# abmoRobotics/isaac_rover_2.0

Hardware: AMD Instinct MI355X
Metric: env-steps/sec (obs+reward+done) (higher is better)
Workload: dtype f32; 1 GPU; BASELINE configs[2]: 65536 envs/GPU x 1 GPU, 37-point heightmap + 26 rock rays, K=200, 600x600 cells @0.1 m, stone_info mask over 1024 stones, cell_index_mode=cuda_rcp; envs_total=65536, rays_per_env=63, obs_dim=41, algorithmic_bytes_per_env_step=227148

## Files before the change

isaac_rover_2.0_amd/csrc/rover_kernels.hip:

```cpp
#include <hip/hip_runtime.h>
#include <stdint.h>
#include <type_traits>
#include "rover_internal.h"
#include "rover_philox.h"
#include "rover_raymath.h"

namespace rover {


__device__ __forceinline__ float quat_roll(const float* __restrict__ q) {
    float w = q[0], x = q[1], y = q[2], z = q[3];
    float sinr = 2.0f * (w * x + y * z);
    float cosr = 1.0f - (2.0f * (x * x + y * y));
    return atan2f(sinr, cosr);
}
__device__ __forceinline__ float quat_pitch(const float* __restrict__ q) {
    const float half_pi = 3.1415927410125732f / 2.0f;
    float w = q[0], x = q[1], y = q[2], z = q[3];
    float sinp = 2.0f * (w * y - z * x);
    float t = sinp - 1.0f;
    return (t >= 0.0f) ? copysignf(half_pi, sinp) : asinf(sinp);
}
__device__ __forceinline__ float quat_yaw(const float* __restrict__ q) {
    float w = q[0], x = q[1], y = q[2], z = q[3];
// ... 736 lines not shown
    float alpha = (float)(2 * 3.14159265358979323846) * u;
    float gx = radius * cosf(alpha) + 0.0f, gy = radius * sinf(alpha) + 0.0f;
    x = gx + initial_pos3[3ull * id];
    y = gy + initial_pos3[3ull * id + 1];
}

__device__ __forceinline__ float height_at(const HeightDev& h, float x, float y) {
    uint32_t ix = cell_coord(x, h.shift_x, h.hscale, h.inv_hscale, h.rcp, h.N0);
    uint32_t iy = cell_coord(y, h.shift_y, h.hscale, h.inv_hscale, h.rcp, h.N0);
    if (iy > (uint32_t)(h.N1 - 1)) iy = (uint32_t)(h.N1 - 1);
    return h.hm[(uint64_t)ix * h.N1 + iy] * h.vscale;
}

#define GOAL_LANES 8u

__global__ void __launch_bounds__(256) goals_draw_kernel(GoalArgs a) {
    const uint32_t n = a.n_dev ? (uint32_t)max(*a.n_dev, 0) : a.n_host;
    const uint32_t gt = blockIdx.x * 256u + threadIdx.x;
    const uint32_t i = gt / GOAL_LANES, j = gt % GOAL_LANES;
    const uint32_t shift = (threadIdx.x & 63u) & ~(GOAL_LANES - 1u);
    const bool live = i < n;
    const int64_t id = live ? a.env_ids[i] - a.id_offset : 0;
    if (live && id == 0 && j == 0) a.t_acc[i] = -1;
    bool active = live && id != 0;
    for (int32_t t0 = 0; t0 < a.max_draws; t0 += (int32_t)GOAL_LANES) {
        if (__builtin_amdgcn_ballot_w64(active) == 0) break;
        const int32_t t = t0 + (int32_t)j;
        bool clear = false;
        float x = 0.0f, y = 0.0f;
        if (active && t < a.max_draws) {
            float u = a.draws ? a.draws[(uint64_t)t * n + i] : philox_uniform(a.seed + (a.seed_dev ? *a.seed_dev : 0ull), (uint32_t)t, (uint32_t)a.env_ids[i]);
            goal_from_draw(u, a.radius, a.initial_pos3, id, x, y);
            clear = !collides_grid(a.grid, a.info7, x, y, 1.0f);
        }
        const uint32_t m = (uint32_t)(__builtin_amdgcn_ballot_w64(clear) >> shift) & ((1u << GOAL_LANES) - 1u);
        if (active) {
            const bool last_trip = t0 + (int32_t)GOAL_LANES >= a.max_draws;
            int32_t winner = -1;
            if (m) winner = (int32_t)__builtin_ctz(m);
            else if (last_trip) winner = a.max_draws - 1 - t0;
            if (winner >= 0) {
                if ((int32_t)j == winner) {
                    a.t_acc[i] = m ? t : a.max_draws;
                    a.target3[3ull * id] = x; a.target3[3ull * id + 1] = y;
                    a.target3[3ull * id + 2] = height_at(a.h, x, y);
                }
                active = false;
            }
        }
    }
}

__global__ void __launch_bounds__(1024) goals_env0_kernel(GoalArgs a) {
    __shared__ int s_tmax, s_lz, s_has_zero, s_fail;
    const uint32_t tid = threadIdx.x;
    const uint32_t n = a.n_dev ? (uint32_t)max(*a.n_dev, 0) : a.n_host;
    if (n == 0) { if (tid == 0 && a.n_draws_used) *a.n_draws_used = 0; return; }
    if (tid == 0) { s_tmax = -1; s_lz = -1; s_has_zero = 0; s_fail = 0; }
    __syncthreads();
    int my_tmax = -1;
    bool my_zero = false, my_fail = false;
    for (uint32_t i = tid; i < n; i += blockDim.x) {
        int32_t t = a.t_acc[i];
        if (t >= a.max_draws) my_fail = true;
        else if (t < 0) my_zero = true;
        else my_tmax = max(my_tmax, t);
    }
#pragma unroll
    for (int o = 32; o >= 1; o >>= 1) my_tmax = max(my_tmax, __shfl_xor(my_tmax, o));
    const bool w_zero = __builtin_amdgcn_ballot_w64(my_zero) != 0, w_fail = __builtin_amdgcn_ballot_w64(my_fail) != 0;
    if ((tid & 63u) == 0u) {
        if (my_tmax >= 0) atomicMax(&s_tmax, my_tmax);
        if (w_zero) s_has_zero = 1;
        if (w_fail) s_fail = 1;
    }
    __syncthreads();
    if (s_fail) { if (tid == 0 && a.n_draws_used) *a.n_draws_used = -1; return; }
    const int tmax = s_tmax;
    int my_lz = -1;
    for (uint32_t i = tid; i < n; i += blockDim.x) {
        int32_t t = a.t_acc[i];
        if (t < 0 || t < tmax) my_lz = max(my_lz, (int)i);
    }
#pragma unroll
    for (int o = 32; o >= 1; o >>= 1) my_lz = max(my_lz, __shfl_xor(my_lz, o));
    if ((tid & 63u) == 0u && my_lz >= 0) atomicMax(&s_lz, my_lz);
    __syncthreads();
    if (tid >= 64u) return;
    const int32_t t0 = max(tmax, 0);
    const int lz0 = s_lz;
    int32_t used = -1;
    float x = 0.0f, y = 0.0f;
    bool wrote = false;
    if (lz0 < 0) {
        used = t0 + 1;
    } else {
        for (int32_t base = t0; base < a.max_draws; base += 64) {
            const int32_t t = base + (int32_t)tid;
            const uint32_t src = (t == t0) ? (uint32_t)lz0 : n - 1u;
            bool clear = false;
            float cx = 0.0f, cy = 0.0f;
            if (t < a.max_draws) {
                float u = a.draws ? a.draws[(uint64_t)t * n + src] : philox_uniform(a.seed + (a.seed_dev ? *a.seed_dev : 0ull), (uint32_t)t, (uint32_t)a.env_ids[src]);
                goal_from_draw(u, a.radius, a.initial_pos3, 0, cx, cy);
                clear = !collides_grid(a.grid, a.info7, cx, cy, 1.0f);
            }
            const uint64_t m = __builtin_amdgcn_ballot_w64(clear);
            const bool last_trip = base + 64 >= a.max_draws;
            int32_t winner = -1;
            if (m) winner = (int32_t)__builtin_ctzll(m);
            else if (last_trip) winner = a.max_draws - 1 - base;
            if (winner >= 0) {
                x = __shfl(cx, winner); y = __shfl(cy, winner);
                wrote = true;
                if (m) used = base + winner + 1;
                break;
            }
        }
    }
    if (tid != 0) return;
    if (wrote) {
        a.target3[0] = x; a.target3[1] = y;
        if (s_has_zero) a.target3[2] = height_at(a.h, x, y);
    }
    if (a.n_draws_used) *a.n_draws_used = used;
}

__global__ void __launch_bounds__(256) reset_envs_kernel(ResetArgs a) {
    const uint32_t n = a.n_dev ? (uint32_t)max(*a.n_dev, 0) : a.n_host;
    uint32_t i = blockIdx.x * blockDim.x + threadIdx.x;
    if (i >= n) return;
    const int64_t id = a.ids[i] - a.id_offset;
    float deg = a.yaw_deg ? (float)a.yaw_deg[i]
                          : floorf(philox_uniform((a.seed + (a.seed_dev ? *a.seed_dev : 0ull)) ^ 0x9E3779B97F4A7C15ull, 0u, (uint32_t)a.ids[i]) * 361.0f);
    float half = (deg * (3.14159265358979323846f / 180.0f)) / 2.0f;
    a.quat4[4ull * id] = sinf(half); a.quat4[4ull * id + 1] = 0.0f; a.quat4[4ull * id + 2] = 0.0f; a.quat4[4ull * id + 3] = cosf(half);
#pragma unroll
    for (int c = 0; c < 3; ++c) {
        float v = a.initial_pos3[3ull * id + c];
        a.pos3[3ull * id + c] = v;
        if (a.base_pos3) a.base_pos3[3ull * id + c] = v;
    }
    for (int j = 0; j < 13; ++j) {
        if (a.joint_pos13) a.joint_pos13[13ull * id + j] = 0.0f;
        if (a.joint_vel13) a.joint_vel13[13ull * id + j] = 0.0f;
    }
    a.reset[id] = 0;
    a.progress[id] = 0;
}

__global__ void __launch_bounds__(256) pre_physics_kernel(PrePhysicsArgs a) {
    uint32_t e = blockIdx.x * blockDim.x + threadIdx.x;
    if (e >= a.E) return;
    if (a.euler_pre) {
        float r, p, y;
        quat_to_euler(a.quat + 4ull * e, r, p, y);
        a.euler_pre[3ull * e] = r; a.euler_pre[3ull * e + 1] = p; a.euler_pre[3ull * e + 2] = y;
    }
    float lin = a.actions[2ull * e], ang = a.actions[2ull * e + 1];
    float l0 = a.lin_hist[3ull * e], l1 = a.lin_hist[3ull * e + 1];
    a.lin_hist[3ull * e] = lin; a.lin_hist[3ull * e + 1] = l0; a.lin_hist[3ull * e + 2] = l1;
    float g0 = a.ang_hist[3ull * e], g1 = a.ang_hist[3ull * e + 1];
    a.ang_hist[3ull * e] = ang; a.ang_hist[3ull * e + 1] = g0; a.ang_hist[3ull * e + 2] = g1;
    if (a.actions_nn) {
        float* n = a.actions_nn + 6ull * e;
        const float n0 = n[0], n1 = n[1], n3 = n[3], n4 = n[4];
        n[0] = lin; n[1] = n0; n[2] = n1; n[3] = ang; n[4] = n3; n[5] = n4;
    }
    if (!a.pos_targets13 && !a.vel_targets13) return;
    const float wl[6][2] = {{-0.385, 0.438}, {0.385, 0.438}, {-0.447, 0.0}, {0.447, 0.0}, {-0.385, -0.411}, {0.385, -0.411}};
    const float side[6] = {-1.0f, 1.0f, -1.0f, 1.0f, -1.0f, 1.0f};
    float Px = copysignf(lin / ang, -ang);
    Px = (fabsf(Px) > 0.45f) ? Px : 0.0f;
    lin = (Px != 0.0f) ? lin : 0.0f;
    float steer[6], vel[6];
#pragma unroll
    for (int w = 0; w < 6; ++w) {
        float dx = Px - wl[w][0], dy = 0.0f - wl[w][1];
        float dist = sqrtf(dx * dx + dy * dy);
        float av = (lin != 0.0f) ? copysignf(ang, lin) : ang * side[w];
        float mv = dist * av;
        if (dist > 1000.0f) mv = lin;
        vel[w] = mv / 0.2f;
        float sa = atan2f(wl[w][1], wl[w][0] - Px);
        if (sa < (float)(-3.14 / 2)) sa = sa + 3.14159265358979323846f;
        if (sa > (float)(3.14 / 2)) sa = sa - 3.14159265358979323846f;
        steer[w] = sa;
    }
    if (a.pos_targets13) {
        float* p = a.pos_targets13 + 13ull * e;
        p[6] = steer[1]; p[8] = steer[5]; p[4] = steer[0]; p[7] = steer[4];
    }
    if (a.vel_targets13) {
        float* v = a.vel_targets13 + 13ull * e;
        v[10] = vel[1]; v[5] = vel[3]; v[12] = vel[5]; v[9] = vel[0]; v[3] = vel[2]; v[11] = vel[4];
    }
}

__global__ void __launch_bounds__(256) ackermann_kernel(const float* __restrict__ lin_in, const float* __restrict__ ang_in,
                                                        uint32_t n, float* __restrict__ steer, float* __restrict__ vel) {
    const float wl[6][2] = {{-0.385, 0.438}, {0.385, 0.438}, {-0.447, 0.0}, {0.447, 0.0}, {-0.385, -0.411}, {0.385, -0.411}};
    const float side[6] = {-1.0f, 1.0f, -1.0f, 1.0f, -1.0f, 1.0f};
    uint32_t i = blockIdx.x * blockDim.x + threadIdx.x;
    if (i >= n) return;
    float lin = lin_in[i], ang = ang_in[i];
    float Px = copysignf(lin / ang, -ang);
    Px = (fabsf(Px) > 0.45f) ? Px : 0.0f;
    lin = (Px != 0.0f) ? lin : 0.0f;
#pragma unroll
    for (int w = 0; w < 6; ++w) {
        float dx = Px - wl[w][0], dy = 0.0f - wl[w][1];
        float dist = sqrtf(dx * dx + dy * dy);
        float av = (lin != 0.0f) ? copysignf(ang, lin) : ang * side[w];
        float mv = dist * av;
        if (dist > 1000.0f) mv = lin;
        vel[6ull * i + w] = mv / 0.2f;
        float sa = atan2f(wl[w][1], wl[w][0] - Px);
        if (sa < (float)(-3.14 / 2)) sa = sa + 3.14159265358979323846f;
        if (sa > (float)(3.14 / 2)) sa = sa - 3.14159265358979323846f;
        steer[6ull * i + w] = sa;
    }
}

#define SCAN_ITEMS 8
#define SCAN_BLOCK 256
#define SCAN_TILE (SCAN_ITEMS * SCAN_BLOCK)

template <int NW>
__device__ __forceinline__ uint32_t block_exclusive_scan(uint32_t v, uint32_t* lds , uint32_t& total) {
    const uint32_t lane = threadIdx.x & 63u, w = threadIdx.x >> 6;
    uint32_t inc = v;
#pragma unroll
    for (int off = 1; off < 64; off <<= 1) {
        uint32_t o = __shfl_up(inc, off, 64);
        if (lane >= (uint32_t)off) inc += o;
    }
    if (lane == 63u) lds[w] = inc;
    __syncthreads();
    uint32_t wbase = 0, tot = 0;
#pragma unroll
    for (int i = 0; i < NW; ++i) { uint32_t c = lds[i]; wbase += ((uint32_t)i < w) ? c : 0u; tot += c; }
    __syncthreads();
    total = tot;
    return wbase + inc - v;
}

__global__ void __launch_bounds__(SCAN_BLOCK) scan_block_sums_kernel(const uint32_t* __restrict__ cnt, uint32_t n,
                                                                     uint32_t* __restrict__ block_sums) {
    __shared__ uint32_t lds[SCAN_BLOCK / 64];
    uint32_t base = blockIdx.x * SCAN_TILE + threadIdx.x * SCAN_ITEMS, sum = 0;
#pragma unroll
    for (int i = 0; i < SCAN_ITEMS; ++i) sum += (base + i < n) ? cnt[base + i] : 0u;
    uint32_t total;
    (void)block_exclusive_scan<SCAN_BLOCK / 64>(sum, lds, total);
    if (threadIdx.x == 0) block_sums[blockIdx.x] = total;
}

__global__ void __launch_bounds__(1024) scan_top_kernel(uint32_t* __restrict__ block_sums, uint32_t nb) {
    __shared__ uint32_t lds[16];
    uint32_t base = threadIdx.x * SCAN_ITEMS, v[SCAN_ITEMS], sum = 0;
#pragma unroll
    for (int i = 0; i < SCAN_ITEMS; ++i) { v[i] = (base + i < nb) ? block_sums[base + i] : 0u; sum += v[i]; }
    uint32_t total, run = block_exclusive_scan<16>(sum, lds, total);
#pragma unroll
    for (int i = 0; i < SCAN_ITEMS; ++i) { if (base + i < nb) block_sums[base + i] = run; run += v[i]; }
}

__global__ void __launch_bounds__(SCAN_BLOCK) scan_apply_kernel(uint32_t* __restrict__ cnt, uint32_t n,
                                                                const uint32_t* __restrict__ block_offsets) {
    __shared__ uint32_t lds[SCAN_BLOCK / 64];
    uint32_t base = blockIdx.x * SCAN_TILE + threadIdx.x * SCAN_ITEMS, v[SCAN_ITEMS], sum = 0;
#pragma unroll
    for (int i = 0; i < SCAN_ITEMS; ++i) { v[i] = (base + i < n) ? cnt[base + i] : 0u; sum += v[i]; }
    uint32_t total, run = block_exclusive_scan<SCAN_BLOCK / 64>(sum, lds, total) + block_offsets[blockIdx.x];
#pragma unroll
    for (int i = 0; i < SCAN_ITEMS; ++i) { if (base + i < n) cnt[base + i] = run; run += v[i]; }
}

#define BKT_ITEMS 16
#define BKT_TILE (256 * BKT_ITEMS)
#define BKT_MAX 4096
#define BKT_STAGE 8192u

template <int NT>
__global__ void __launch_bounds__(NT) bucket_hist_kernel(const uint32_t* __restrict__ bins, uint32_t n_slots, uint32_t low_bits,
                                                          uint32_t n_buckets, uint32_t n_blocks, uint32_t* __restrict__ counts) {
    __shared__ uint32_t h[BKT_MAX];
    for (uint32_t i = threadIdx.x; i < n_buckets; i += NT) h[i] = 0;
    __syncthreads();
    const uint32_t base = blockIdx.x * (NT * BKT_ITEMS);
    uint32_t bv[BKT_ITEMS];
#pragma unroll
    for (uint32_t it = 0; it < BKT_ITEMS; ++it) {
        const uint32_t i = base + it * NT + threadIdx.x;
        bv[it] = i < n_slots ? bins[i] : 0xffffffffu;
    }
#pragma unroll
    for (uint32_t it = 0; it < BKT_ITEMS; ++it)
        if (bv[it] != 0xffffffffu) atomicAdd(&h[bv[it] >> low_bits], 1u);
    __syncthreads();
    for (uint32_t i = threadIdx.x; i < n_buckets; i += NT) counts[(size_t)blockIdx.x * n_buckets + i] = h[i];
}

#define RSCAN_WAVES 16
__global__ void __launch_bounds__(64 * RSCAN_WAVES) bucket_rowscan_kernel(uint32_t* __restrict__ counts, uint32_t n_blocks, uint32_t n_buckets,
                                                                          uint32_t* __restrict__ bucket_tot) {
    __shared__ uint32_t part[RSCAN_WAVES][16];
    const uint32_t lane = threadIdx.x & 63u, w = threadIdx.x >> 6, kb = lane & 15u, ph = lane >> 4;
    const uint32_t k = blockIdx.x * 16u + kb;
    const bool kin = k < n_buckets;
    uint32_t carry = 0;
    for (uint32_t tile0 = 0; tile0 < n_blocks; tile0 += 64u * RSCAN_WAVES) {
        const uint32_t b0 = tile0 + w * 64u + ph;
        uint32_t* __restrict__ p = counts + (size_t)b0 * n_buckets + (kin ? k : 0u);
        uint32_t v[16], ex[16], sum = 0;
#pragma unroll
        for (uint32_t j = 0; j < 16u; ++j) v[j] = (kin && b0 + 4u * j < n_blocks) ? p[(size_t)(4u * j) * n_buckets] : 0u;
#pragma unroll
        for (uint32_t j = 0; j < 16u; ++j) {
            uint32_t inc = v[j];
            uint32_t o = (uint32_t)__shfl_up((int)inc, 16, 64); if (ph >= 1u) inc += o;
            o = (uint32_t)__shfl_up((int)inc, 32, 64);          if (ph >= 2u) inc += o;
            const uint32_t four = (uint32_t)__shfl((int)inc, 48 + (int)kb, 64);
            ex[j] = sum + inc - v[j];
            sum += four;
        }
        if (ph == 0u) part[w][kb] = sum;
        __syncthreads();
        uint32_t run = carry, total = 0;
#pragma unroll
        for (uint32_t i = 0; i < RSCAN_WAVES; ++i) { const uint32_t c = part[i][kb]; run += i < w ? c : 0u; total += c; }
        __syncthreads();
#pragma unroll
        for (uint32_t j = 0; j < 16u; ++j)
            if (kin && b0 + 4u * j < n_blocks) p[(size_t)(4u * j) * n_buckets] = run + ex[j];
        carry += total;
    }
    if (w == 0 && ph == 0u && kin) bucket_tot[k] = carry;
}

template <bool PACKED> struct BktEntry;
template <> struct BktEntry<false> {
    typedef uint2 T;
    static __device__ __forceinline__ T make(uint32_t bin, uint32_t slot, uint32_t) { return make_uint2(bin, slot); }
    static __device__ __forceinline__ T none() { return make_uint2(0u, 0xffffffffu); }
    static __device__ __forceinline__ uint32_t lo(T v, uint32_t low_bits) { return v.x & ((1u << low_bits) - 1u); }
    static __device__ __forceinline__ uint32_t slot(T v, uint32_t) { return v.y; }
};
template <> struct BktEntry<true> {
    typedef uint32_t T;
    static __device__ __forceinline__ T make(uint32_t bin, uint32_t slot, uint32_t low_bits) { return (bin << (32u - low_bits)) | slot; }
    static __device__ __forceinline__ T none() { return 0xffffffffu; }
    static __device__ __forceinline__ uint32_t lo(T v, uint32_t low_bits) { return v >> (32u - low_bits); }
    static __device__ __forceinline__ uint32_t slot(T v, uint32_t low_bits) { return v & (0xffffffffu >> low_bits); }
};

template <bool PACKED, int NT>
__global__ void __launch_bounds__(NT) bucket_scatter_kernel(const uint32_t* __restrict__ bins, uint32_t n_slots, uint32_t low_bits,
                                                             uint32_t n_buckets, uint32_t n_blocks, const uint32_t* __restrict__ offsets,
                                                             const uint32_t* __restrict__ bucket_tot, uint32_t* __restrict__ bucket_base,
                                                             uint2* __restrict__ pairs2) {
    typedef BktEntry<PACKED> En;
    typename En::T* __restrict__ pairs = reinterpret_cast<typename En::T*>(pairs2);
    extern __shared__ __attribute__((aligned(8))) uint32_t bkt_lds[];
    uint32_t* const cur = bkt_lds;
    uint32_t* const cnt = cur + n_buckets;
    uint32_t* const s_dst = cnt + n_buckets;
    typename En::T* const s_val = reinterpret_cast<typename En::T*>(s_dst + (NT * BKT_ITEMS));
    __shared__ uint32_t wl[NT / 64];
    const uint32_t per = (n_buckets + NT - 1u) / NT, first = threadIdx.x * per;
    const uint32_t base = blockIdx.x * (NT * BKT_ITEMS);
    uint32_t bv[BKT_ITEMS], rk[BKT_ITEMS];
#pragma unroll
    for (uint32_t it = 0; it < BKT_ITEMS; ++it) {
        const uint32_t i = base + it * NT + threadIdx.x;
        bv[it] = i < n_slots ? bins[i] : 0xffffffffu;
    }
    {
        uint32_t sum = 0;
        for (uint32_t j = 0; j < per; ++j) sum += (first + j < n_buckets) ? bucket_tot[first + j] : 0u;
        uint32_t total, run = block_exclusive_scan<NT / 64>(sum, wl, total);
        for (uint32_t j = 0; j < per; ++j) {
            const uint32_t i = first + j;
            if (i < n_buckets) {
                cur[i] = run + offsets[(size_t)blockIdx.x * n_buckets + i];
                cnt[i] = 0u;
                if (blockIdx.x == 0) bucket_base[i] = run;
                run += bucket_tot[i];
            }
        }
        if (blockIdx.x == 0 && threadIdx.x == 0) bucket_base[n_buckets] = total;
    }
    __syncthreads();
#pragma unroll
    for (uint32_t it = 0; it < BKT_ITEMS; ++it) rk[it] = bv[it] != 0xffffffffu ? atomicAdd(&cnt[bv[it] >> low_bits], 1u) : 0u;
    __syncthreads();
    uint32_t n_here;
    {
        uint32_t sum = 0;
        for (uint32_t j = 0; j < per; ++j) sum += (first + j < n_buckets) ? cnt[first + j] : 0u;
        uint32_t run = block_exclusive_scan<NT / 64>(sum, wl, n_here);
        for (uint32_t j = 0; j < per; ++j) {
            const uint32_t i = first + j;
            if (i < n_buckets) { const uint32_t c = cnt[i]; cnt[i] = run; run += c; }
        }
    }
    __syncthreads();
#pragma unroll
    for (uint32_t it = 0; it < BKT_ITEMS; ++it) {
        if (bv[it] != 0xffffffffu) {
            const uint32_t b = bv[it] >> low_bits, l = cnt[b] + rk[it];
            s_dst[l] = cur[b] + rk[it];
            s_val[l] = En::make(bv[it], base + it * NT + threadIdx.x, low_bits);
        }
    }
    __syncthreads();
    for (uint32_t k = threadIdx.x; k < n_here; k += NT) pairs[s_dst[k]] = s_val[k];
}

template <bool PACKED, int NT, int IPT>
__global__ void __launch_bounds__(NT) bucket_sort_kernel(const uint2* __restrict__ pairs2, const uint32_t* __restrict__ bucket_base,
                                                          uint32_t low_bits, uint32_t* __restrict__ sorted, uint32_t* __restrict__ zero,
                                                          uint32_t n_zero) {
    typedef BktEntry<PACKED> En;
    const typename En::T* __restrict__ pairs = reinterpret_cast<const typename En::T*>(pairs2);
    extern __shared__ uint32_t bkt_lds[];
    __shared__ uint32_t wl[NT / 64];
    const uint32_t b = blockIdx.x, tid = threadIdx.x, nl = 1u << low_bits;
    if (zero) {
        const uint32_t per = (n_zero + gridDim.x - 1u) / gridDim.x, z1 = min(n_zero, (b + 1u) * per);
        for (uint32_t i = b * per + tid; i < z1; i += NT) zero[i] = 0u;
    }
    uint32_t* const h = bkt_lds;
    uint32_t* const stage = bkt_lds + nl;
    const uint32_t s0 = bucket_base[b], s1 = bucket_base[b + 1u];
    if (s1 <= s0) return;
    for (uint32_t i = tid; i < nl; i += NT) h[i] = 0;
    __syncthreads();
    if (s1 - s0 <= (uint32_t)(NT * IPT)) {
        uint32_t slot[IPT], br[IPT];
#pragma unroll
        for (int g = 0; g < IPT / 8; ++g) {
            typename En::T pv[8];
#pragma unroll
            for (int j = 0; j < 8; ++j) { const uint32_t k = s0 + tid + (uint32_t)(8 * g + j) * NT; pv[j] = k < s1 ? pairs[k] : En::none(); }
#pragma unroll
            for (int j = 0; j < 8; ++j) {
                const uint32_t k = s0 + tid + (uint32_t)(8 * g + j) * NT, lo = En::lo(pv[j], low_bits);
                slot[8 * g + j] = En::slot(pv[j], low_bits);
                br[8 * g + j] = k < s1 ? (lo | (atomicAdd(&h[lo], 1u) << 12)) : 0u;
            }
        }
        __syncthreads();
        const uint32_t per = (nl + NT - 1u) / NT, first = tid * per;
        uint32_t sum = 0;
        for (uint32_t j = 0; j < per; ++j) sum += first + j < nl ? h[first + j] : 0u;
        uint32_t total, run = block_exclusive_scan<NT / 64>(sum, wl, total);
        for (uint32_t j = 0; j < per; ++j) if (first + j < nl) { const uint32_t c = h[first + j]; h[first + j] = run; run += c; }
        __syncthreads();
        if (s1 - s0 <= BKT_STAGE) {
#pragma unroll
            for (int i = 0; i < IPT; ++i) {
                const uint32_t k = s0 + tid + (uint32_t)i * NT;
                if (k < s1) stage[h[br[i] & 0xfffu] + (br[i] >> 12)] = slot[i];
            }
            __syncthreads();
            for (uint32_t k = tid; k < s1 - s0; k += NT) sorted[s0 + k] = stage[k];
            return;
        }
#pragma unroll
        for (int i = 0; i < IPT; ++i) {
            const uint32_t k = s0 + tid + (uint32_t)i * NT;
            if (k < s1) sorted[s0 + h[br[i] & 0xfffu] + (br[i] >> 12)] = slot[i];
        }
        return;
    }
    for (uint32_t k0 = s0 + tid; k0 < s1; k0 += 8u * NT) {
        typename En::T bx[8];
#pragma unroll
        for (int j = 0; j < 8; ++j) { const uint32_t k = k0 + (uint32_t)j * NT; bx[j] = k < s1 ? pairs[k] : En::none(); }
#pragma unroll
        for (int j = 0; j < 8; ++j) if (k0 + (uint32_t)j * NT < s1) atomicAdd(&h[En::lo(bx[j], low_bits)], 1u);
    }
    __syncthreads();
    const uint32_t per = (nl + NT - 1u) / NT, first = tid * per;
    uint32_t sum = 0;
    for (uint32_t j = 0; j < per; ++j) sum += first + j < nl ? h[first + j] : 0u;
    uint32_t total, run = block_exclusive_scan<NT / 64>(sum, wl, total);
    for (uint32_t j = 0; j < per; ++j) if (first + j < nl) { const uint32_t c = h[first + j]; h[first + j] = run; run += c; }
    __syncthreads();
    for (uint32_t k0 = s0 + tid; k0 < s1; k0 += 8u * NT) {
        typename En::T pv[8];
#pragma unroll
        for (int j = 0; j < 8; ++j) { const uint32_t k = k0 + (uint32_t)j * NT; pv[j] = k < s1 ? pairs[k] : En::none(); }
#pragma unroll
        for (int j = 0; j < 8; ++j)
            if (k0 + (uint32_t)j * NT < s1) sorted[s0 + atomicAdd(&h[En::lo(pv[j], low_bits)], 1u)] = En::slot(pv[j], low_bits);
    }
}

template <int H>
__global__ void __launch_bounds__(256) raycast_binned_kernel(const RayRec* __restrict__ rays, const uint32_t* __restrict__ sorted,
                                                             uint32_t n_sorted, const _Float16* __restrict__ tab0,
                                                             const _Float16* __restrict__ tab1, uint32_t kp0, uint32_t kp1,
                                                             uint32_t run, uint32_t n_blocks, uint32_t nb8,
                                                             uint32_t pre_terrain, uint32_t pre_rocks, float* __restrict__ out) {
    const uint32_t lb = (blockIdx.x & 7u) * nb8 + (blockIdx.x >> 3);
    if (lb >= n_blocks) return;
    const uint32_t wave = __builtin_amdgcn_readfirstlane(lb * 4u + (threadIdx.x >> 6));
    const uint32_t lane = threadIdx.x & 63u;
    uint32_t i = wave * run;
    if (i >= n_sorted) return;
    const uint32_t i_end = min(i + run, n_sorted);
    uint32_t cur_cell = 0xffffffffu, cur_map = 0xffffffffu;
    std::conditional_t<H != 0, CellRegsH<2>, CellRegs<2>> t;
    t.poison();
    uint64_t vmask[2][2] = {{0, 0}, {0, 0}};
    for (; i < i_end; ++i) {
        const uint32_t gid = __builtin_amdgcn_readfirstlane(sorted[i]);
        const float4* rp = reinterpret_cast<const float4*>(rays + gid);
        const float4 ra = rp[0], rb = rp[1];
        const uint32_t cell = __builtin_amdgcn_readfirstlane(__float_as_uint(ra.w));
        const uint32_t map = __builtin_amdgcn_readfirstlane(__float_as_uint(rb.w)) & 1u;
        if (cell != cur_cell || map != cur_map) {
            if (map != cur_map && cur_map != 0xffffffffu && kp0 != kp1) t.poison();
            cur_cell = cell; cur_map = map;
            const uint32_t kp = map ? kp1 : kp0;
            const _Float16* base = (map ? tab1 : tab0) + (size_t)cell * 9u * kp + lane * 4u;
            if (lane * 4u < kp) {
                half4 v[9];
#pragma unroll
                for (int q = 0; q < 9; ++q) v[q] = *reinterpret_cast<const half4*>(base + (size_t)q * kp);
#pragma unroll
                for (int p = 0; p < 2; ++p) {
                    const int t0 = 2 * p, t1 = 2 * p + 1;
                    if constexpr (H) {
                        h2 vv[9];
#pragma unroll
                        for (int q = 0; q < 9; ++q) vv[q] = h2{v[q][t0], v[q][t1]};
                        set_pair_h(t, p, vv);
                    } else {
                        f2 w[9];
#pragma unroll
                        for (int q = 0; q < 9; ++q) w[q] = f2{(float)v[q][t0], (float)v[q][t1]};
                        set_pair(t, p, w);
                    }
                }
            }
#pragma unroll
            for (int p = 0; p < 2; ++p) {
                vmask[p][0] = __builtin_amdgcn_ballot_w64(t.ax[p].x == t.ax[p].x);
                vmask[p][1] = __builtin_amdgcn_ballot_w64(t.ax[p].y == t.ax[p].y);
            }
        }
        float best;
        if constexpr (H) {
            const _Float16 hsx = (_Float16)ra.x, hsy = (_Float16)ra.y, hsz = (_Float16)ra.z;
            const _Float16 hdx = (_Float16)rb.x, hdy = (_Float16)rb.y, hdz = (_Float16)rb.z;
            best = cast_pairs_h<2>(t, h2{hsx, hsx}, h2{hsy, hsy}, h2{hsz, hsz}, h2{hdx, hdx}, h2{hdy, hdy}, h2{hdz, hdz}, vmask,
                                   map ? pre_rocks : pre_terrain);
        } else {
            const f2 sx = {ra.x, ra.x}, sy = {ra.y, ra.y}, sz = {ra.z, ra.z};
            const f2 dx = {rb.x, rb.x}, dy = {rb.y, rb.y}, dz = {rb.z, rb.z};
            best = cast_pairs<2>(t, sx, sy, sz, dx, dy, dz, vmask, map ? pre_rocks : pre_terrain);
        }
        best = wave_min_to_lane63(best);
        if (lane == 63u) out[gid] = best;
    }
}

#define KNN_CAP 8192

__global__ void __launch_bounds__(256) knn_centroid_kernel(const float* __restrict__ verts, const int32_t* __restrict__ tris,
                                                           uint32_t T, uint32_t V, int ref, float* __restrict__ cx, float* __restrict__ cy) {
    uint32_t t = blockIdx.x * blockDim.x + threadIdx.x;
    if (t >= T) return;
    uint32_t a = (uint32_t)tris[3ull * t], b = (uint32_t)tris[3ull * t + 1], c = (uint32_t)tris[3ull * t + 2];
    a = a < V ? a : 0u; b = b < V ? b : 0u; c = c < V ? c : 0u;
    if (ref) {
        double x = (((double)verts[3ull * a] + (double)verts[3ull * b]) + (double)verts[3ull * c]) / 3.0;
        double y = (((double)verts[3ull * a + 1] + (double)verts[3ull * b + 1]) + (double)verts[3ull * c + 1]) / 3.0;
        cx[t] = (float)(_Float16)(float)x;
        cy[t] = (float)(_Float16)(float)y;
        return;
    }
    cx[t] = (verts[3ull * a] + verts[3ull * b] + verts[3ull * c]) / 3.0f;
    cy[t] = (verts[3ull * a + 1] + verts[3ull * b + 1] + verts[3ull * c + 1]) / 3.0f;
}

__device__ __forceinline__ uint32_t knn_bucket(float v, float origin, float inv_g, uint32_t n) {
    float f = (v - origin) * inv_g;
    if (!(f > 0.0f)) return 0u;
    uint32_t b = (uint32_t)f;
    return b < n ? b : n - 1u;
}

__global__ void __launch_bounds__(256) knn_bucket_kernel(const float* __restrict__ cx, const float* __restrict__ cy, uint32_t T,
                                                         float ox, float oy, float inv_g, uint32_t nbx, uint32_t nby,
                                                         uint32_t* __restrict__ cursor, uint32_t* __restrict__ items, int count) {
    uint32_t t = blockIdx.x * blockDim.x + threadIdx.x;
    if (t >= T) return;
    uint32_t b = knn_bucket(cx[t], ox, inv_g, nbx) * nby + knn_bucket(cy[t], oy, inv_g, nby);
    uint32_t pos = atomicAdd(cursor + b, 1u);
    if (!count) items[pos] = t;
}

__global__ void __launch_bounds__(256) knn_select_kernel(const float* __restrict__ cx, const float* __restrict__ cy,
                                                         const uint32_t* __restrict__ bucket_start, const uint32_t* __restrict__ items,
                                                         float ox, float oy, float g, uint32_t nbx, uint32_t nby, uint32_t X,
                                                         uint32_t Y, float res, uint32_t K, const float* __restrict__ cell_x,
                                                         const float* __restrict__ cell_y, int32_t* __restrict__ out,
                                                         int32_t* __restrict__ overflow) {
    __shared__ unsigned long long keys[KNN_CAP];
    __shared__ uint32_t count;
    const uint32_t cell = blockIdx.x, x = cell / Y, y = cell % Y, tid = threadIdx.x;
    const bool ref = cell_x != nullptr;
    const float px = ref ? cell_x[x] : (float)x * res, py = ref ? cell_y[y] : (float)y * res;
    const float inv_g = 1.0f / g;
    const int bx = (int)knn_bucket(px, ox, inv_g, nbx), by = (int)knn_bucket(py, oy, inv_g, nby);
    const int rmax = (int)max(nbx, nby);
    if (tid == 0) count = 0;
    __syncthreads();
    for (int r = 0; r <= rmax; ++r) {
        const int side = 2 * r + 1, nring = r == 0 ? 1 : 8 * r;
        for (int q = (int)tid; q < nring; q += 256) {
            int i, j;
            if (r == 0) { i = bx; j = by; }
            else if (q < side) { i = bx - r; j = by - r + q; }
            else if (q < 2 * side) { i = bx + r; j = by - r + (q - side); }
            else if (q < 2 * side + (side - 2)) { i = bx - r + 1 + (q - 2 * side); j = by - r; }
            else { i = bx - r + 1 + (q - 2 * side - (side - 2)); j = by + r; }
            if (i < 0 || j < 0 || i >= (int)nbx || j >= (int)nby) continue;
            const uint32_t b = (uint32_t)i * nby + (uint32_t)j, s0 = bucket_start[b], s1 = bucket_start[b + 1];
            if (s1 == s0) continue;
            uint32_t base = atomicAdd(&count, s1 - s0);
            for (uint32_t k = s0; k < s1; ++k, ++base) {
                if (base >= KNN_CAP) break;
                const uint32_t t = items[k];
                float dx = cx[t] - px, dy = cy[t] - py;
                if (ref) { dx = (float)(_Float16)dx; dy = (float)(_Float16)dy; }
                const float d2 = dx * dx + dy * dy;
                const float key = ref ? (float)(_Float16)sqrtf(d2) : d2;
                keys[base] = ((unsigned long long)__float_as_uint(key) << 32) | t;
            }
        }
        __syncthreads();
        const uint32_t n = count;
        __syncthreads();
        if (n > KNN_CAP) { if (tid == 0) *overflow = 1; return; }
        const bool covers_all = (bx - r <= 0) && (by - r <= 0) && (bx + r >= (int)nbx - 1) && (by + r >= (int)nby - 1);
        if (n >= K || covers_all) {
            uint32_t m = 1; while (m < n) m <<= 1;
            for (uint32_t k = n + tid; k < m; k += 256) keys[k] = ~0ull;
            __syncthreads();
            for (uint32_t len = 2; len <= m; len <<= 1) {
                for (uint32_t stride = len >> 1; stride > 0; stride >>= 1) {
                    for (uint32_t k = tid; k < (m >> 1); k += 256) {
                        const uint32_t lo = ((k / stride) * stride << 1) + (k % stride), hi = lo + stride;
                        const bool up = ((lo & len) == 0);
                        const unsigned long long a = keys[lo], b = keys[hi];
                        if ((a > b) == up) { keys[lo] = b; keys[hi] = a; }
                    }
                    __syncthreads();
                }
            }
            const float reach = (float)r * g;
            const float kth = n >= K ? __uint_as_float((uint32_t)(keys[K - 1] >> 32)) : __builtin_inff();
            if (covers_all || (ref ? kth < reach * (1.0f - 1.0f / 512.0f) : kth <= reach * reach)) {
                for (uint32_t k = tid; k < K; k += 256) out[(uint64_t)cell * K + k] = k < n ? (int32_t)(uint32_t)keys[k] : 0;
                return;
            }
            __syncthreads();
        }
    }
}

hipError_t launch_repack(const int32_t* map_idx, const int32_t* tris, const uint16_t* verts, uint64_t n_cells, uint32_t K,
                         uint32_t K8, uint32_t T, uint32_t V, uint16_t* table, hipStream_t s) {
    uint64_t n = n_cells * K8;
    hipLaunchKernelGGL(repack_knn_kernel, dim3(blocks_for(n, 256)), dim3(256), 0, s, map_idx, tris, verts, n_cells, K, K8, T, V, table);
    return hipGetLastError();
}

hipError_t launch_prep(const PrepArgs& a, hipStream_t s) {
    const uint32_t target = (a.hist && a.hist_buckets > 576u) ? 2048u : 1024u;
    const uint32_t xb = blocks_for(a.E, 64), n_groups = a.R8 / PREP_SLOTS;
    const uint32_t yb = max(1u, min(n_groups, (target + xb - 1u) / xb)), gpb = (n_groups + yb - 1u) / yb;
    hipLaunchKernelGGL(prep_rays_kernel, dim3(xb, (n_groups + gpb - 1u) / gpb), dim3(64 * PREP_SLOTS), a.hist ? a.hist_buckets * 4u : 0u, s, a, gpb);
    return hipGetLastError();
}

hipError_t launch_raycast(const RayRec* rays, uint32_t n_rays, const uint16_t* tab0, const uint16_t* tab1, uint32_t kp0,
                          uint32_t kp1, float* out, hipStream_t s) {
    hipLaunchKernelGGL(raycast_kernel, dim3(blocks_for(n_rays, 8)), dim3(256), 0, s, rays, n_rays,
                       reinterpret_cast<const _Float16*>(tab0), reinterpret_cast<const _Float16*>(tab1), kp0, kp1, out);
    return hipGetLastError();
}

hipError_t launch_scan_exclusive(uint32_t* data, uint32_t n, uint32_t* block_sums, hipStream_t s);

bool bin_entries_packed(uint32_t n_slots, uint32_t low_bits) { return (uint64_t)n_slots <= (1ull << (32u - low_bits)); }
static inline uint32_t bin_tile_threads(uint32_t n_slots, bool packed) {
    const bool big = n_slots >= (2u << 20);
    return big ? (packed ? 1024u : 512u) : 256u;
}

bool bin_hist_fused(uint32_t n_slots, uint32_t R8, uint32_t n_bins, uint32_t low_bits, uint32_t* blocks_per_tile) {
    const uint32_t n_buckets = (n_bins + (1u << low_bits) - 1u) >> low_bits;
    const uint32_t tile = bin_tile_threads(n_slots, bin_entries_packed(n_slots, low_bits)) * BKT_ITEMS, keys = 64u * R8;
    if (low_bits < 8u || low_bits > 12u || n_buckets > 1024u || keys > tile || tile % keys != 0u) return false;
    *blocks_per_tile = tile / keys;
    return true;
}

hipError_t launch_bin_rays(const uint32_t* bins, uint32_t n_slots, uint32_t n_valid, uint32_t n_bins, uint32_t low_bits, bool packed,
                           uint32_t* table, uint2* pairs, uint32_t* block_sums, uint32_t* sorted, bool hist_done, hipStream_t s) {
    const uint32_t n_buckets = (n_bins + (1u << low_bits) - 1u) >> low_bits;
    if (low_bits < 8u || low_bits > 12u || n_buckets > BKT_MAX) return hipErrorInvalidValue;
    const bool big = n_slots >= (2u << 20);
    if (packed != bin_entries_packed(n_slots, low_bits)) return hipErrorInvalidValue;
    const uint32_t nt = bin_tile_threads(n_slots, packed), tile = nt * BKT_ITEMS;
    const uint32_t n_blocks = blocks_for(n_slots, tile);
    uint32_t* bucket_tot = block_sums;
    uint32_t* const zero = hist_done ? table : nullptr;
    const uint32_t n_zero = n_blocks * n_buckets;
    uint32_t* bucket_base = block_sums + BKT_MAX;
    const uint32_t scatter_lds = (2u * n_buckets + (packed ? 2u : 3u) * tile + 2u) * 4u, sort_lds = ((1u << low_bits) + BKT_STAGE) * 4u;
#define BKT_LAUNCH(PK, NT)                                                                                                            \
    do {                                                                                                                              \
        if (!hist_done) hipLaunchKernelGGL(bucket_hist_kernel<NT>, dim3(n_blocks), dim3(NT), 0, s, bins, n_slots, low_bits, n_buckets, n_blocks, table); \
        hipLaunchKernelGGL(bucket_rowscan_kernel, dim3(blocks_for(n_buckets, 16)), dim3(64 * RSCAN_WAVES), 0, s, table, n_blocks, n_buckets, bucket_tot); \
        hipLaunchKernelGGL((bucket_scatter_kernel<PK, NT>), dim3(n_blocks), dim3(NT), scatter_lds, s, bins, n_slots, low_bits, n_buckets, n_blocks, \
                           table, bucket_tot, bucket_base, pairs);                                                                   \
         \
        if ((uint64_t)n_valid > 8192ull * n_buckets)                                                                                  \
            hipLaunchKernelGGL((bucket_sort_kernel<PK, 1024, 32>), dim3(n_buckets), dim3(1024), sort_lds, s, pairs, bucket_base, low_bits, sorted, zero, n_zero); \
        else                                                                                                                          \
            hipLaunchKernelGGL((bucket_sort_kernel<PK, 512, 32>), dim3(n_buckets), dim3(512), sort_lds, s, pairs, bucket_base, low_bits, sorted, zero, n_zero);     \
    } while (0)
    if (big) {
        static uint32_t raised_of[64][2] = {};
        int dev = 0;
        if (hipGetDevice(&dev) != hipSuccess || dev < 0 || dev >= 64) dev = 0;
        uint32_t* raised = raised_of[dev];
        if (scatter_lds > raised[packed]) {
            const void* f = packed ? reinterpret_cast<const void*>(&bucket_scatter_kernel<true, 1024>) : reinterpret_cast<const void*>(&bucket_scatter_kernel<false, 512>);
            const hipError_t e = hipFuncSetAttribute(f, hipFuncAttributeMaxDynamicSharedMemorySize, (int)scatter_lds);
            if (e != hipSuccess) return e;
            raised[packed] = scatter_lds;
        }
    }
    if (packed) { if (big) BKT_LAUNCH(true, 1024); else BKT_LAUNCH(true, 256); }
    else { if (big) BKT_LAUNCH(false, 512); else BKT_LAUNCH(false, 256); }
#undef BKT_LAUNCH
    return hipGetLastError();
}

hipError_t launch_raycast_binned(const RayRec* rays, const uint32_t* sorted, uint32_t n_sorted, const uint16_t* tab0,
                                 const uint16_t* tab1, uint32_t kp0, uint32_t kp1, uint32_t run, bool fp16_math, uint32_t early_out,
                                 float* out, hipStream_t s) {
    const uint32_t n_waves = blocks_for(n_sorted, run);
    const uint32_t n_blocks = blocks_for(n_waves, 4);
    const uint32_t nb8 = blocks_for(n_blocks, 8);
    const _Float16* t0 = reinterpret_cast<const _Float16*>(tab0);
    const _Float16* t1 = reinterpret_cast<const _Float16*>(tab1);
    const uint32_t pre_terrain = early_out ? 2u : 0u, pre_rocks = early_out ? 3u : 0u;
    if (fp16_math)
        hipLaunchKernelGGL(raycast_binned_kernel<1>, dim3(nb8 * 8u), dim3(256), 0, s, rays, sorted, n_sorted, t0, t1, kp0, kp1, run,
                           n_blocks, nb8, pre_terrain, pre_rocks, out);
    else
        hipLaunchKernelGGL(raycast_binned_kernel<0>, dim3(nb8 * 8u), dim3(256), 0, s, rays, sorted, n_sorted, t0, t1, kp0, kp1, run,
                           n_blocks, nb8, pre_terrain, pre_rocks, out);
    return hipGetLastError();
}

hipError_t launch_knn_centroids(const float* verts, const int32_t* tris, uint32_t T, uint32_t V, int ref, float* cx, float* cy,
                                hipStream_t s) {
    hipLaunchKernelGGL(knn_centroid_kernel, dim3(blocks_for(T, 256)), dim3(256), 0, s, verts, tris, T, V, ref, cx, cy);
    return hipGetLastError();
}

hipError_t launch_knn_bucket(const float* cx, const float* cy, uint32_t T, float ox, float oy, float inv_g, uint32_t nbx, uint32_t nby,
                             uint32_t* cursor, uint32_t* items, int count, hipStream_t s) {
    hipLaunchKernelGGL(knn_bucket_kernel, dim3(blocks_for(T, 256)), dim3(256), 0, s, cx, cy, T, ox, oy, inv_g, nbx, nby, cursor, items,
                       count);
    return hipGetLastError();
}

hipError_t launch_scan_exclusive(uint32_t* data, uint32_t n, uint32_t* block_sums, hipStream_t s) {
    const uint32_t nb = blocks_for(n, SCAN_TILE);
    if (nb > 1024u * SCAN_ITEMS) return hipErrorInvalidValue;
    hipLaunchKernelGGL(scan_block_sums_kernel, dim3(nb), dim3(SCAN_BLOCK), 0, s, data, n, block_sums);
    hipLaunchKernelGGL(scan_top_kernel, dim3(1), dim3(1024), 0, s, block_sums, nb);
    hipLaunchKernelGGL(scan_apply_kernel, dim3(nb), dim3(SCAN_BLOCK), 0, s, data, n, block_sums);
    return hipGetLastError();
}

hipError_t launch_knn_select(const float* cx, const float* cy, const uint32_t* bucket_start, const uint32_t* items, float ox, float oy,
                             float g, uint32_t nbx, uint32_t nby, uint32_t X, uint32_t Y, float res, uint32_t K, const float* cell_x,
                             const float* cell_y, int32_t* out, int32_t* overflow, hipStream_t s) {
    hipLaunchKernelGGL(knn_select_kernel, dim3(X * Y), dim3(256), 0, s, cx, cy, bucket_start, items, ox, oy, g, nbx, nby, X, Y, res, K,
                       cell_x, cell_y, out, overflow);
    return hipGetLastError();
}

hipError_t launch_assemble_obs(const ObsArgs& a_in, hipStream_t s) {
    ObsArgs a = a_in;
    a.w_div = make_fastdiv(a.W);
    hipLaunchKernelGGL(assemble_obs_kernel, dim3(blocks_for((uint64_t)a.E * a.W, 256 * OBS_ILP)), dim3(256), 0, s, a);
    return hipGetLastError();
}

hipError_t launch_export_dist(const float* dist, const RayRec* rays, uint32_t E, uint32_t R8, uint32_t P, int precision, float* ray_dist,
                              float* wheel, float* body, float* ray_src, float* hit_pt, hipStream_t s) {
    hipLaunchKernelGGL(export_dist_kernel, dim3(blocks_for((uint64_t)E * (26u + P), 256)), dim3(256), 0, s, dist, rays, E, R8, P, precision,
                       ray_dist, wheel, body, ray_src, hit_pt);
    return hipGetLastError();
}

hipError_t launch_export_rays(const RayRec* rays, const float* dist, uint32_t E, uint32_t R8, uint32_t P, float* src, float* dir, int32_t* cell,
                              float* out_dist, hipStream_t s) {
    hipLaunchKernelGGL(export_rays_kernel, dim3(blocks_for((uint64_t)E * (26u + P), 256)), dim3(256), 0, s, rays, dist, E, R8, 26u + P, src, dir,
                       cell, out_dist);
    return hipGetLastError();
}

hipError_t launch_import_rays(const float* src, const float* dir, uint32_t E, uint32_t R8, uint32_t P, const KnnDev& terrain, const KnnDev& rocks,
                              uint32_t rocks_bin_offset, int precision, int cell_rcp, RayRec* rays, uint32_t* bin_out, hipStream_t s,
                              uint32_t* not_unit) {
    hipLaunchKernelGGL(import_rays_kernel, dim3(blocks_for((uint64_t)E * R8, 256)), dim3(256), 0, s, src, dir, E, R8, 26u + P, terrain, rocks,
                       rocks_bin_offset, precision, cell_rcp, rays, bin_out, not_unit);
    return hipGetLastError();
}

hipError_t launch_obs_metrics(const ObsArgs& o_in, const MetricsArgs& m, hipStream_t s) {
    ObsArgs o = o_in;
    o.w_div = make_fastdiv(o.W);
    const uint32_t n_met = blocks_for(m.E, 256), n_obs = blocks_for((uint64_t)o.E * o.W, 256 * OBS_ILP);
    hipLaunchKernelGGL(obs_metrics_kernel, dim3(n_met + n_obs), dim3(256), 0, s, o, m, n_met);
    return hipGetLastError();
}

hipError_t launch_metrics_done(const MetricsArgs& a, hipStream_t s) {
    hipLaunchKernelGGL(metrics_done_kernel, dim3(blocks_for(a.E, 256)), dim3(256), 0, s, a);
    return hipGetLastError();
}

hipError_t launch_compact(const int64_t* reset, uint32_t n, int64_t offset, uint32_t* block_cnt, bool counted, int64_t* ids,
                          int32_t* count, hipStream_t s) {
    const uint32_t nb = blocks_for(n, 256);
    if (!counted) hipLaunchKernelGGL(compact_count_kernel, dim3(nb), dim3(256), 0, s, reset, n, block_cnt);
    hipLaunchKernelGGL(compact_write_kernel, dim3(nb), dim3(256), 0, s, reset, n, offset, block_cnt, ids, count);
    return hipGetLastError();
}

hipError_t launch_eval_summary(const int64_t* eval_res, const int64_t* eval_step, uint32_t E, int64_t* summary8, hipStream_t s) {
    hipError_t err = hipMemsetAsync(summary8, 0, 8 * sizeof(int64_t), s);
    if (err != hipSuccess) return err;
    uint32_t nb = blocks_for(E, 256);
    if (nb > 1024u) nb = 1024u;
    hipLaunchKernelGGL(eval_summary_kernel, dim3(nb), dim3(256), 0, s, eval_res, eval_step, E,
                       reinterpret_cast<unsigned long long*>(summary8));
    return hipGetLastError();
}

hipError_t launch_eval_clear(int64_t* eval_res, int64_t* eval_step, uint32_t E, const int64_t* ids, uint32_t n, hipStream_t s) {
    if (n == 0) return hipSuccess;
    hipLaunchKernelGGL(eval_clear_kernel, dim3(blocks_for(n, 256)), dim3(256), 0, s, eval_res, eval_step, E, ids, n);
    return hipGetLastError();
}

hipError_t launch_quat_to_euler(const float* q, float* eul, uint32_t n, hipStream_t s) {
    hipLaunchKernelGGL(quat_to_euler_kernel, dim3(blocks_for(n, 256)), dim3(256), 0, s, q, eul, n);
    return hipGetLastError();
}

hipError_t launch_clearance(const float* info7, uint32_t S, const float* xy, uint32_t n, float* out, hipStream_t s) {
    hipLaunchKernelGGL(clearance_kernel, dim3(blocks_for(n, 256)), dim3(256), 0, s, info7, S, xy, n, out);
    return hipGetLastError();
}

hipError_t launch_shift_spawns(const StoneGridDev& g, const float* info7, float* pos3, uint32_t n, int32_t max_iter, hipStream_t s) {
    hipLaunchKernelGGL(shift_spawns_kernel, dim3(blocks_for(n, 256)), dim3(256), 0, s, g, info7, pos3, n, max_iter);
    return hipGetLastError();
}

hipError_t launch_sample_height(const HeightDev& h, const float* xy, uint32_t n, float* out, hipStream_t s) {
    hipLaunchKernelGGL(sample_height_kernel, dim3(blocks_for(n, 256)), dim3(256), 0, s, h, xy, n, out);
    return hipGetLastError();
}

hipError_t launch_generate_goals(const GoalArgs& a, uint32_t n_max, hipStream_t s) {
    hipLaunchKernelGGL(goals_draw_kernel, dim3(blocks_for((uint64_t)n_max * GOAL_LANES, 256)), dim3(256), 0, s, a);
    hipLaunchKernelGGL(goals_env0_kernel, dim3(1), dim3(1024), 0, s, a);
    return hipGetLastError();
}

hipError_t launch_reset_envs(const ResetArgs& a, uint32_t n_max, hipStream_t s) {
    hipLaunchKernelGGL(reset_envs_kernel, dim3(blocks_for(n_max, 256)), dim3(256), 0, s, a);
    return hipGetLastError();
}

hipError_t launch_pre_physics(const PrePhysicsArgs& a, hipStream_t s) {
    hipLaunchKernelGGL(pre_physics_kernel, dim3(blocks_for(a.E, 256)), dim3(256), 0, s, a);
    return hipGetLastError();
}

hipError_t launch_ackermann(const float* lin, const float* ang, uint32_t n, float* steer, float* vel, hipStream_t s) {
    hipLaunchKernelGGL(ackermann_kernel, dim3(blocks_for(n, 256)), dim3(256), 0, s, lin, ang, n, steer, vel);
    return hipGetLastError();
}

}
```

Before: 167.7 million env-steps/s.

## Reshape bucket row-scan, cache offsets in scatter, prefetch pairs in bucket sort

The row-scan kernel now uses 4 waves with 4 buckets per block and 4 rows per lane instead of 16x16, which launches more blocks and uses fewer registers per thread. The scatter kernel reads bucket totals and offsets once into LDS, so it no longer re-reads global memory in the second pass. The bucket sort kernel loads pairs into registers before the histogram zeroing, overlapping that load with the LDS clear. It also drops the packed br encoding in favour of a separate rank array, which may raise register pressure with IPT=32.

Measured after the change: 168.2 million env-steps/s (median of 6 runs). No clear change (+0.3%).

```diff
diff --git a/isaac_rover_2.0_amd/csrc/rover_kernels.hip b/isaac_rover_2.0_amd/csrc/rover_kernels.hip
--- a/isaac_rover_2.0_amd/csrc/rover_kernels.hip
+++ b/isaac_rover_2.0_amd/csrc/rover_kernels.hip
@@ -1062,28 +1062,34 @@
     for (uint32_t i = threadIdx.x; i < n_buckets; i += NT) counts[(size_t)blockIdx.x * n_buckets + i] = h[i];
 }
 
-#define RSCAN_WAVES 16
+#define RSCAN_WAVES 4
+#define RSCAN_KB 4u
+#define RSCAN_PH (64u / RSCAN_KB)
+#define RSCAN_J 4u
 __global__ void __launch_bounds__(64 * RSCAN_WAVES) bucket_rowscan_kernel(uint32_t* __restrict__ counts, uint32_t n_blocks, uint32_t n_buckets,
                                                                           uint32_t* __restrict__ bucket_tot) {
-    __shared__ uint32_t part[RSCAN_WAVES][16];
-    const uint32_t lane = threadIdx.x & 63u, w = threadIdx.x >> 6, kb = lane & 15u, ph = lane >> 4;
-    const uint32_t k = blockIdx.x * 16u + kb;
+    __shared__ uint32_t part[RSCAN_WAVES][RSCAN_KB];
+    const uint32_t lane = threadIdx.x & 63u, w = threadIdx.x >> 6, kb = lane & (RSCAN_KB - 1u), ph = lane / RSCAN_KB;
+    const uint32_t k = blockIdx.x * RSCAN_KB + kb;
     const bool kin = k < n_buckets;
     uint32_t carry = 0;
-    for (uint32_t tile0 = 0; tile0 < n_blocks; tile0 += 64u * RSCAN_WAVES) {
-        const uint32_t b0 = tile0 + w * 64u + ph;
+    for (uint32_t tile0 = 0; tile0 < n_blocks; tile0 += RSCAN_WAVES * RSCAN_J * RSCAN_PH) {
+        const uint32_t b0 = tile0 + w * (RSCAN_J * RSCAN_PH) + ph;
         uint32_t* __restrict__ p = counts + (size_t)b0 * n_buckets + (kin ? k : 0u);
-        uint32_t v[16], ex[16], sum = 0;
-#pragma unroll
-        for (uint32_t j = 0; j < 16u; ++j) v[j] = (kin && b0 + 4u * j < n_blocks) ? p[(size_t)(4u * j) * n_buckets] : 0u;
-#pragma unroll
-        for (uint32_t j = 0; j < 16u; ++j) {
+        uint32_t v[RSCAN_J], ex[RSCAN_J], sum = 0;
+#pragma unroll
+        for (uint32_t j = 0; j < RSCAN_J; ++j) v[j] = (kin && b0 + RSCAN_PH * j < n_blocks) ? p[(size_t)(RSCAN_PH * j) * n_buckets] : 0u;
+#pragma unroll
+        for (uint32_t j = 0; j < RSCAN_J; ++j) {
             uint32_t inc = v[j];
-            uint32_t o = (uint32_t)__shfl_up((int)inc, 16, 64); if (ph >= 1u) inc += o;
-            o = (uint32_t)__shfl_up((int)inc, 32, 64);          if (ph >= 2u) inc += o;
-            const uint32_t four = (uint32_t)__shfl((int)inc, 48 + (int)kb, 64);
+#pragma unroll
+            for (uint32_t d = 1u; d < RSCAN_PH; d <<= 1) {
+                const uint32_t o = (uint32_t)__shfl_up((int)inc, (int)(d * RSCAN_KB), 64);
+                if (ph >= d) inc += o;
+            }
+            const uint32_t all = (uint32_t)__shfl((int)inc, (int)(64u - RSCAN_KB + kb), 64);
             ex[j] = sum + inc - v[j];
-            sum += four;
+            sum += all;
         }
         if (ph == 0u) part[w][kb] = sum;
         __syncthreads();
@@ -1092,8 +1098,8 @@
         for (uint32_t i = 0; i < RSCAN_WAVES; ++i) { const uint32_t c = part[i][kb]; run += i < w ? c : 0u; total += c; }
         __syncthreads();
 #pragma unroll
-        for (uint32_t j = 0; j < 16u; ++j)
-            if (kin && b0 + 4u * j < n_blocks) p[(size_t)(4u * j) * n_buckets] = run + ex[j];
+        for (uint32_t j = 0; j < RSCAN_J; ++j)
+            if (kin && b0 + RSCAN_PH * j < n_blocks) p[(size_t)(RSCAN_PH * j) * n_buckets] = run + ex[j];
         carry += total;
     }
     if (w == 0 && ph == 0u && kin) bucket_tot[k] = carry;
@@ -1137,16 +1143,21 @@
         bv[it] = i < n_slots ? bins[i] : 0xffffffffu;
     }
     {
+        const uint32_t* __restrict__ const row = offsets + (size_t)blockIdx.x * n_buckets;
         uint32_t sum = 0;
-        for (uint32_t j = 0; j < per; ++j) sum += (first + j < n_buckets) ? bucket_tot[first + j] : 0u;
+        for (uint32_t j = 0; j < per; ++j) {
+            const uint32_t i = first + j;
+            if (i < n_buckets) { const uint32_t t = bucket_tot[i]; cur[i] = row[i]; cnt[i] = t; sum += t; }
+        }
         uint32_t total, run = block_exclusive_scan<NT / 64>(sum, wl, total);
         for (uint32_t j = 0; j < per; ++j) {
             const uint32_t i = first + j;
             if (i < n_buckets) {
-                cur[i] = run + offsets[(size_t)blockIdx.x * n_buckets + i];
+                const uint32_t t = cnt[i];
+                cur[i] += run;
                 cnt[i] = 0u;
                 if (blockIdx.x == 0) bucket_base[i] = run;
-                run += bucket_tot[i];
+                run += t;
             }
         }
         if (blockIdx.x == 0 && threadIdx.x == 0) bucket_base[n_buckets] = total;
@@ -1195,21 +1206,26 @@
     uint32_t* const stage = bkt_lds + nl;
     const uint32_t s0 = bucket_base[b], s1 = bucket_base[b + 1u];
     if (s1 <= s0) return;
+    const uint32_t n = s1 - s0;
+    const bool one_pass = n <= (uint32_t)(NT * IPT);
+    typename En::T pv[IPT];
+    if (one_pass) {
+#pragma unroll
+        for (int i = 0; i < IPT; ++i) {
+            if ((uint32_t)i * NT >= n) break;
+            const uint32_t k = tid + (uint32_t)i * NT;
+            pv[i] = k < n ? pairs[s0 + k] : En::none();
+        }
+    }
     for (uint32_t i = tid; i < nl; i += NT) h[i] = 0;
     __syncthreads();
-    if (s1 - s0 <= (uint32_t)(NT * IPT)) {
-        uint32_t slot[IPT], br[IPT];
-#pragma unroll
-        for (int g = 0; g < IPT / 8; ++g) {
-            typename En::T pv[8];
-#pragma unroll
-            for (int j = 0; j < 8; ++j) { const uint32_t k = s0 + tid + (uint32_t)(8 * g + j) * NT; pv[j] = k < s1 ? pairs[k] : En::none(); }
-#pragma unroll
-            for (int j = 0; j < 8; ++j) {
-                const uint32_t k = s0 + tid + (uint32_t)(8 * g + j) * NT, lo = En::lo(pv[j], low_bits);
-                slot[8 * g + j] = En::slot(pv[j], low_bits);
-                br[8 * g + j] = k < s1 ? (lo | (atomicAdd(&h[lo], 1u) << 12)) : 0u;
-            }
+    if (one_pass) {
+        uint32_t rk[IPT];
+#pragma unroll
+        for (int i = 0; i < IPT; ++i) {
+            if ((uint32_t)i * NT >= n) break;
+            if ((uint32_t)(i + 1) * NT <= n) rk[i] = atomicAdd(&h[En::lo(pv[i], low_bits)], 1u);
+            else rk[i] = tid + (uint32_t)i * NT < n ? atomicAdd(&h[En::lo(pv[i], low_bits)], 1u) : 0u;
         }
         __syncthreads();
         const uint32_t per = (nl + NT - 1u) / NT, first = tid * per;
@@ -1218,20 +1234,20 @@
         uint32_t total, run = block_exclusive_scan<NT / 64>(sum, wl, total);
         for (uint32_t j = 0; j < per; ++j) if (first + j < nl) { const uint32_t c = h[first + j]; h[first + j] = run; run += c; }
         __syncthreads();
-        if (s1 - s0 <= BKT_STAGE) {
+        if (n <= BKT_STAGE) {
 #pragma unroll
             for (int i = 0; i < IPT; ++i) {
-                const uint32_t k = s0 + tid + (uint32_t)i * NT;
-                if (k < s1) stage[h[br[i] & 0xfffu] + (br[i] >> 12)] = slot[i];
+                if ((uint32_t)i * NT >= n) break;
+                if (tid + (uint32_t)i * NT < n) stage[h[En::lo(pv[i], low_bits)] + rk[i]] = En::slot(pv[i], low_bits);
             }
             __syncthreads();
-            for (uint32_t k = tid; k < s1 - s0; k += NT) sorted[s0 + k] = stage[k];
+            for (uint32_t k = tid; k < n; k += NT) sorted[s0 + k] = stage[k];
             return;
         }
 #pragma unroll
         for (int i = 0; i < IPT; ++i) {
-            const uint32_t k = s0 + tid + (uint32_t)i * NT;
-            if (k < s1) sorted[s0 + h[br[i] & 0xfffu] + (br[i] >> 12)] = slot[i];
+            if ((uint32_t)i * NT >= n) break;
+            if (tid + (uint32_t)i * NT < n) sorted[s0 + h[En::lo(pv[i], low_bits)] + rk[i]] = En::slot(pv[i], low_bits);
         }
         return;
     }
@@ -1250,12 +1266,12 @@
     for (uint32_t j = 0; j < per; ++j) if (first + j < nl) { const uint32_t c = h[first + j]; h[first + j] = run; run += c; }
     __syncthreads();
     for (uint32_t k0 = s0 + tid; k0 < s1; k0 += 8u * NT) {
-        typename En::T pv[8];
-#pragma unroll
-        for (int j = 0; j < 8; ++j) { const uint32_t k = k0 + (uint32_t)j * NT; pv[j] = k < s1 ? pairs[k] : En::none(); }
+        typename En::T px[8];
+#pragma unroll
+        for (int j = 0; j < 8; ++j) { const uint32_t k = k0 + (uint32_t)j * NT; px[j] = k < s1 ? pairs[k] : En::none(); }
 #pragma unroll
         for (int j = 0; j < 8; ++j)
-            if (k0 + (uint32_t)j * NT < s1) sorted[s0 + atomicAdd(&h[En::lo(pv[j], low_bits)], 1u)] = En::slot(pv[j], low_bits);
+            if (k0 + (uint32_t)j * NT < s1) sorted[s0 + atomicAdd(&h[En::lo(px[j], low_bits)], 1u)] = En::slot(px[j], low_bits);
     }
 }
 
@@ -1489,7 +1505,7 @@
 #define BKT_LAUNCH(PK, NT)                                                                                                            \
     do {                                                                                                                              \
         if (!hist_done) hipLaunchKernelGGL(bucket_hist_kernel<NT>, dim3(n_blocks), dim3(NT), 0, s, bins, n_slots, low_bits, n_buckets, n_blocks, table); \
-        hipLaunchKernelGGL(bucket_rowscan_kernel, dim3(blocks_for(n_buckets, 16)), dim3(64 * RSCAN_WAVES), 0, s, table, n_blocks, n_buckets, bucket_tot); \
+        hipLaunchKernelGGL(bucket_rowscan_kernel, dim3(blocks_for(n_buckets, RSCAN_KB)), dim3(64 * RSCAN_WAVES), 0, s, table, n_blocks, n_buckets, bucket_tot); \
         hipLaunchKernelGGL((bucket_scatter_kernel<PK, NT>), dim3(n_blocks), dim3(NT), scatter_lds, s, bins, n_slots, low_bits, n_buckets, n_blocks, \
                            table, bucket_tot, bucket_base, pairs);                                                                   \
          \
```
